# williamfgc/ROCm-MPI

Hardware: AMD Instinct MI355X
Metric: T_eff (GB/s) + weak-scaling eff., 2D diffusion 1000 steps at 1/2/4/8 MI355X (higher is better)
Workload: dtype fp64

## Files before the change

csrc/bindings/module.cpp:

```cpp
#include <pybind11/pybind11.h>
#include <pybind11/stl.h>

#include <cstdint>
#include <string>
#include <tuple>
#include <vector>

#include "rma/config.h"
#include "rma/comm.h"
#include "rma/common.h"
#include "rma/executor.h"
#include "rma/executor3d.h"
#include "rma/gather.h"
#include "rma/halo.h"
#include "rma/ipc.h"
#include "rma/kernels.h"
#include "rma/loopback.h"
#include "rma/p2p.h"
#include "rma/plan.h"
#include "rma/topology.h"
#include "rma/trace.h"

namespace py = pybind11;
using namespace rma;
// ... 134 lines not shown
        else {
          py::gil_scoped_release nogil;
          stencil2_rects_cpu(P<double>(T2), P<const double>(T), P<const double>(iCp), nx, ny,
                             r.data(), (int)r.size(), to_coef(coef));
        }
      },
      py::arg("T2"), py::arg("T"), py::arg("iCp"), py::arg("nx"), py::arg("ny"), py::arg("rects"),
      py::arg("coef"), py::arg("chunk_rows") = 8, py::arg("nontemporal") = 3,
      py::arg("stream") = 0, py::arg("gpu") = true, py::arg("unroll") = 2,
      py::arg("xcd_remap") = -1);
  m.def(
      "stencilk_rects",
      [](int K, uintptr_t T2, uintptr_t T, uintptr_t iCp, int64_t nx, int64_t ny,
         const std::vector<Rect4>& rects, const Coef4& coef, int chunk_rows, int nontemporal,
         uintptr_t stream, bool gpu, int xcd_remap, int vec, int kernel, int stages, int cols,
         bool uniform, double uniform_value) {
        auto r = to_rects(rects);
        StencilTuning tn;
        tn.cols = cols;
        tn.uniform = uniform;
        tn.uniform_value = uniform_value;
        tn.chunk_rows = chunk_rows;
        tn.nontemporal = nontemporal;
        tn.xcd_remap = xcd_remap;
        tn.vec = vec;
        tn.kernel = kernel;
        tn.stages = stages;
        if (gpu)
          stencilk_rects_gpu(K, P<double>(T2), P<const double>(T), P<const double>(iCp), nx, ny,
                             r.data(), (int)r.size(), to_coef(coef), tn, S(stream));
        else {
          const bool f5 = (kernel >= 5 && kernel <= 9) || kernel == 12 || kernel == 22;
          py::gil_scoped_release nogil;
          if (f5)
            stencilk5_rects_cpu(K, P<double>(T2), P<const double>(T), P<const double>(iCp), nx,
                                ny, r.data(), (int)r.size(), to_coef(coef));
          else
            stencilk_rects_cpu(K, P<double>(T2), P<const double>(T), P<const double>(iCp), nx,
                               ny, r.data(), (int)r.size(), to_coef(coef));
        }
      },
      py::arg("K"), py::arg("T2"), py::arg("T"), py::arg("iCp"), py::arg("nx"), py::arg("ny"),
      py::arg("rects"), py::arg("coef"), py::arg("chunk_rows") = 16, py::arg("nontemporal") = 3,
      py::arg("stream") = 0, py::arg("gpu") = true, py::arg("xcd_remap") = -1,
      py::arg("vec") = 2, py::arg("kernel") = 0, py::arg("stages") = 0, py::arg("cols") = 0,
      py::arg("uniform") = false, py::arg("uniform_value") = 0.0);
  m.def(
      "stencil3d_boxes",
      [](uintptr_t T2, uintptr_t T, uintptr_t iCp, int64_t nx, int64_t ny, int64_t nz,
         const std::vector<Box6>& boxes, const Coef5& coef, int rows, int unroll, int vec,
         int nontemporal, int chunk_z, int xcd_remap, uintptr_t stream, bool gpu, bool uniform,
         double uniform_value, bool fast_math, int xface) {
        auto b = to_boxes(boxes);
        if (gpu) {
          Stencil3DTuning tn;
          tn.fast_math = fast_math ? 1 : 0;
          tn.xface = xface;
          tn.uniform = uniform;
          tn.uniform_value = uniform_value;
          tn.rows = rows;
          tn.unroll = unroll;
// ... 397 lines not shown
      .def("set_self_via_transport", &HaloExchanger::set_self_via_transport)
      .def_property_readonly("neighbors", &HaloExchanger::neighbors)
      .def_property_readonly("bytes_sent_last", &HaloExchanger::bytes_sent_last)
      .def_property_readonly("plan_hits", &HaloExchanger::plan_hits)
      .def_property_readonly("plan_misses", &HaloExchanger::plan_misses);

  m.def("pipe_chunk_rows", &pipe_chunk_rows, py::arg("K"), py::arg("ny"),
        py::arg("canonical") = false);
  m.def("default_chunk_k", [](int K, int64_t ny) { return default_tune_k(K, ny).chunk_rows; },
        py::arg("K"), py::arg("ny"));
  m.def("plan_passes", &plan_passes, py::arg("nsteps"), py::arg("costs"));
  m.def("uniform_pass_costs", &uniform_pass_costs, py::arg("kmax"), py::arg("cells") = 0.0);
  m.def("pipe_uniform_cells", &pipe_uniform_cells, py::arg("K"), py::arg("cells"));
  m.def("default_pass_costs", &default_pass_costs, py::arg("kmax"), py::arg("fast5"),
        py::arg("cells") = 0.0);
  m.def("pipe_default_stages", &pipe_default_stages, py::arg("K"));
  m.def("pipe_default_cols", &pipe_default_cols, py::arg("K"), py::arg("stages"),
        py::arg("arith") = 0);
  m.def("pipe_has_cols", &pipe_has_cols, py::arg("K"), py::arg("stages"), py::arg("arith"),
        py::arg("cols"));
  m.def("pipe_vec", &pipe_vec, py::arg("K"), py::arg("stages"), py::arg("arith"), py::arg("nx"),
        py::arg("requested"), py::arg("aligned16") = true);
  m.def("pipe_vec_uniform", &pipe_vec_uniform, py::arg("K"), py::arg("stages"), py::arg("arith"),
        py::arg("nx"), py::arg("requested"), py::arg("aligned16") = true,
        py::arg("uniform") = false);
  m.def("pipe_max_k", []() { return kPipeMaxK; });
  m.def(
      "pass_geometry",
      [](int64_t nx, int64_t ny, int K, std::array<std::array<int, 2>, 3> nbr, bool hide,
         int64_t bwx, int64_t bwy, int64_t olx, int64_t oly) {
// ... 61 lines not shown
           py::arg("mode"), py::arg("coef"), py::arg("chunk_rows") = 4,
           py::arg("nontemporal") = 3, py::arg("kernel") = 0, py::arg("bwx") = 1,
           py::arg("bwy") = 1, py::arg("use_graph") = 0, py::arg("graph_steps") = 0,
           py::arg("halo").none(true) = nullptr, py::arg("qx") = 0, py::arg("qy") = 0,
           py::arg("dTdt") = 0, py::arg("unroll") = 4, py::arg("vec") = 2,
           py::arg("temporal") = 1, py::arg("olx") = 2, py::arg("oly") = 2,
           py::arg("chunk2") = 0, py::arg("unroll2") = 2, py::arg("fast_math") = 0,
           py::keep_alive<1, 16>())
      .def(
          "run", [](DiffusionExecutor& e, int64_t n, uintptr_t s) { e.run(n, S(s)); },
          py::arg("nsteps"), py::arg("stream"), py::call_guard<py::gil_scoped_release>())
      .def_property_readonly("parity", &DiffusionExecutor::parity)
      .def_property_readonly("steps_done", &DiffusionExecutor::steps_done)
      .def_property_readonly("passes_done", &DiffusionExecutor::passes_done)
      .def_property_readonly("fused_passes", &DiffusionExecutor::fused_passes)
      .def_property_readonly("uniform_factor", &DiffusionExecutor::uniform_factor)
      .def("rescan_factor", &DiffusionExecutor::rescan_factor,
           py::call_guard<py::gil_scoped_release>())
      .def("check_error", &DiffusionExecutor::check_error)
      .def("plan", &DiffusionExecutor::plan, py::arg("nsteps"))
      .def_property_readonly("pass_costs", &DiffusionExecutor::pass_costs)
      .def("prime", &DiffusionExecutor::prime, py::call_guard<py::gil_scoped_release>())
      .def("set_timing", &DiffusionExecutor::set_timing, py::arg("on"),
           py::call_guard<py::gil_scoped_release>())
      .def("timings",
           [](DiffusionExecutor& e) {
             std::vector<py::dict> out;
             std::vector<PassTiming> ts;
             {
               py::gil_scoped_release nogil;
// ... 151 lines not shown
```

csrc/include/rma/executor.h:

```cpp
#pragma once

#include <array>
#include <cstdint>
#include <memory>
#include <vector>

#include "rma/halo.h"
#include "rma/kernels.h"
#include "rma/plan.h"

namespace rma {

enum class Mode : int { kPerf = 0, kHide = 1, kKp = 2 };

struct ExecParams {
  Mode mode = Mode::kPerf;
  StencilCoef coef{};
  StencilTuning tune{};
  int64_t bwx = 1, bwy = 1;
  int use_graph = 0;
  int graph_steps = 0;
  int temporal = 1;
  int64_t olx = 2, oly = 2;
  StencilTuning tune2{16, 3, 0, 2, 2, -1};
// ... 19 lines not shown
  DiffusionExecutor(const DiffusionExecutor&) = delete;
  DiffusionExecutor& operator=(const DiffusionExecutor&) = delete;

  void run(int64_t nsteps, stream_t caller_stream);
  std::vector<int> plan(int64_t nsteps) const;
  const std::vector<double>& pass_costs() const { return cost_; }
  void prime();
  void set_timing(bool on);
  std::vector<PassTiming> timings();
  void set_solo(bool on);
  bool solo() const { return solo_; }
  int parity() const { return parity_; }
  int64_t steps_done() const { return steps_; }
  int64_t passes_done() const { return passes_; }
  int64_t fused_passes() const { return fused_passes_; }
  void check_error() const { check_fused_error(); }
  bool uniform_factor() const { return uniform_; }
  bool rescan_factor();
  struct DirectPeer {
    int rank = -1;
    double* T = nullptr;
    double* T2 = nullptr;
    uint64_t* flag = nullptr;
  };
  static constexpr int kDirI[8] = {-1, 0, 1, -1, 1, -1, 0, 1};
  static constexpr int kDirJ[8] = {-1, -1, -1, 0, 0, 1, 1, 1};
  void set_direct(const std::array<DirectPeer, 8>& peers, uint64_t* in_flags,
                  bool host_wait = false);
  bool direct() const { return direct_on_; }
  int64_t direct_passes() const { return direct_pass_; }
  std::vector<Rect> frame_rects() const { return frame_; }
  Rect interior_rect() const { return interior_; }
  Rect full_rect() const { return full_; }
  const PassGeom& geometry(int K);

 private:
  void enqueue_step(double* Tin, double* Tout);
  void enqueue_pass(int K, double* Tin, double* Tout);
  StencilTuning pass_tuning(int K, int part = 0) const;
  int frame_chunk_rows(int K, int interior_rows) const;
  void multi_step(int K, double* Tin, double* Tout, const double* iCp, int64_t nx, int64_t ny,
                  const Rect* rects, int n, const StencilTuning& tn, void* stream) const;
  void exchange(double* A, stream_t s);
  bool cross_pass_ = false;
  void build_graph(int64_t steps, int reps);
  void run_eager(int64_t nsteps);
  bool fast5() const;
  void scan_factor();
  bool uniform_ = false;
  double c0_ = 0.0;
  int cells_ = 0;

  double* T_;
  double* T2_;
  const double* iCp_;
  int64_t nx_, ny_;
  ExecParams p_;
// ... 64 lines not shown
```

csrc/include/rma/kernels.h:

```cpp
#pragma once

#include <cstddef>
#include <cstdint>

#include "rma/common.h"

namespace rma {

using stream_t = void*;

constexpr int kMaxRects = 8;

struct DirectStores {
  int on = 0;
  int32_t xm0 = 0, xm1 = 0, xp0 = 0, xp1 = 0;
  int32_t ym0 = 0, ym1 = 0, yp0 = 0, yp1 = 0;
  int64_t sx = 0, syr = 0;
  double* dst[8] = {};
};

struct StencilTuning {
  int chunk_rows = 4;
  int nontemporal = 3;
  int kernel = 0;
  int unroll = 4;
  int vec = 2;
  int xcd_remap = -1;
  int stages = 0;
  int cols = 0;
  uint64_t* signal = nullptr;
  int signal_rects = 0;
  int signal_chunk_rows = 0;
  const DirectStores* direct = nullptr;
  bool uniform = false;
  double uniform_value = 0.0;
};

void stencil_rects_gpu(double* T2, const double* T, const double* iCp, int64_t nx, int64_t ny,
                       const Rect* rects, int nrects, const StencilCoef& c,
                       const StencilTuning& tune, stream_t stream);
void stencil_rects_cpu(double* T2, const double* T, const double* iCp, int64_t nx, int64_t ny,
                       const Rect* rects, int nrects, const StencilCoef& c);

void stencil2_rects_gpu(double* T2, const double* T, const double* iCp, int64_t nx, int64_t ny,
                        const Rect* rects, int nrects, const StencilCoef& c,
                        const StencilTuning& tune, stream_t stream);
void stencil2_rects_cpu(double* T2, const double* T, const double* iCp, int64_t nx, int64_t ny,
// ... 6 lines not shown
                        int64_t ny, const Rect* rects, int nrects, const StencilCoef& c);
bool fast5_ok(const StencilCoef& c);
constexpr int kPipeMaxK = 24;
int pipe_default_stages(int K);
bool pipe_has(int K, int stages, int arith = 0);
bool pipe_has_cols(int K, int stages, int arith, int cols);
int pipe_default_cols(int K, int stages, int arith);
int pipe_vec(int K, int stages, int arith, int64_t nx, int requested, bool aligned16);
int pipe_vec_uniform(int K, int stages, int arith, int64_t nx, int requested, bool aligned16,
                     bool uniform);
void stencil_pipe_occupancy(int K, int stages, int arith, int V, int occ[2]);
void stencil_pipe_rects_gpu(int K, int stages, int arith, double* T2, const double* T,
                            const double* iCp, int64_t nx, int64_t ny, const Rect* rects,
                            int nrects, const StencilCoef& c, const StencilTuning& tune,
                            stream_t stream);
void stencil5_rects_cpu(double* T2, const double* T, const double* iCp, int64_t nx, int64_t ny,
                        const Rect* rects, int nrects, const StencilCoef& c);
void stencilk5_rects_cpu(int K, double* T2, const double* T, const double* iCp, int64_t nx,
                         int64_t ny, const Rect* rects, int nrects, const StencilCoef& c);

void count_differing_gpu(const double* A, int64_t n, uint64_t* out2, stream_t stream);
int64_t count_differing_cpu(const double* A, int64_t n);

constexpr int kMaxBoxes = 8;

struct Stencil3DTuning {
  int rows = 4;
  int unroll = 2;
  int vec = 2;
  int nontemporal = 3;
// ... 151 lines not shown
```

csrc/include/rma/plan.h:

```cpp
#pragma once

#include <array>
#include <cstdint>
#include <vector>

#include "rma/common.h"

namespace rma {

using Neighbors = std::array<std::array<int, 2>, 3>;

void split_rect(const Rect& out, int64_t bwx, int64_t bwy, std::vector<Rect>& frame,
                Rect& interior);
void split_rect_sides(const Rect& out, int64_t xlo, int64_t xhi, int64_t ylo, int64_t yhi,
                      std::vector<Rect>& frame, Rect& interior);

Rect owned_rect(int64_t nx, int64_t ny, int K, const Neighbors& nbr);

std::array<std::array<bool, 2>, 2> frame_sides(const Neighbors& nbr);

struct PassGeom {
  Rect out{};
  std::vector<Rect> frame;
  Rect interior{};
// ... 11 lines not shown
                       int64_t task_h = 0, int vec = 1, int bands = -1, int out_k = 0);

struct FrameLayout {
  int chunk_div = 1;
  int bands = -1;
};
FrameLayout frame_layout(int64_t ny, const Neighbors& nbr);

std::vector<double> default_pass_costs(int kmax, bool fast5, double cells = 0);
std::vector<double> uniform_pass_costs(int kmax, double cells);
int pipe_uniform_cells(int K, double cells);
void apply_cost_overrides(std::vector<double>& cost, const char* spec);

int pipe_chunk_rows(int K, int64_t ny, bool canonical);

std::vector<int> plan_passes(int64_t n, const std::vector<double>& cost);

}
```

csrc/kernels/stencil_device.h:

```cpp
#pragma once

#include <hip/hip_runtime.h>

#include <algorithm>
#include <type_traits>

#include "rma/kernels.h"

namespace rma {
namespace march {

constexpr int kWave = 64;
constexpr int kWavesPerBlock = 4;
constexpr int kBlock = kWave * kWavesPerBlock;
constexpr int64_t kColMaxWidth = 8;
typedef double dbl2 __attribute__((ext_vector_type(2)));
typedef double dbl2u __attribute__((ext_vector_type(2), aligned(8)));

template <int V>
using dbl2v = typename std::conditional<V % 2 == 0, dbl2, dbl2u>::type;

struct RectList {
  Rect r[kMaxRects];
  int64_t xa[kMaxRects];
  int64_t strips[kMaxRects];
  int64_t chunks[kMaxRects];
  int64_t block_end[kMaxRects];
  int64_t gpad[kMaxRects];
  int64_t crows[kMaxRects];
  int n;
  uint64_t* sig;
  int64_t sig_blocks;
};

template <int V, bool NTL = false>
__device__ __forceinline__ void load_row(double (&out)[V], const double* __restrict__ p) {
  if constexpr (V == 1) {
    out[0] = NTL ? __builtin_nontemporal_load(p) : *p;
  } else {
#pragma unroll
    for (int h = 0; h < V / 2; ++h) {
      const dbl2v<V>* q = reinterpret_cast<const dbl2v<V>*>(p + 2 * h);
      const dbl2v<V> t = NTL ? __builtin_nontemporal_load(q) : *q;
      out[2 * h] = t.x;
      out[2 * h + 1] = t.y;
// ... 32 lines not shown
      return;
    }
  }
#pragma unroll
  for (int i = 0; i < V; ++i) {
    if (m[i]) {
      if constexpr (NT) {
        __builtin_nontemporal_store(v[i], p + i);
      } else {
        p[i] = v[i];
      }
    }
  }
}

__device__ __forceinline__ int64_t xcd_remap(int64_t b, int64_t nwg) {
  constexpr int64_t kXcd = 8;
  if (nwg < kXcd) return b;
  const int64_t q = nwg / kXcd, r = nwg % kXcd;
  const int64_t xcd = b % kXcd, slot = b / kXcd;
  return (xcd < r ? xcd * (q + 1) : r * (q + 1) + (xcd - r) * q) + slot;
}

__device__ __forceinline__ int64_t xcd_remap_after(int64_t b, int64_t nwg, int64_t first) {
  return b < first ? b : first + xcd_remap(b - first, nwg - first);
}

__device__ __forceinline__ void signal_block_done(uint64_t* sig, int64_t nblocks) {
  __syncthreads();
  if (threadIdx.x == 0) {
    const uint64_t old =
        __hip_atomic_fetch_add(sig, (uint64_t)1, __ATOMIC_ACQ_REL, __HIP_MEMORY_SCOPE_AGENT);
    if ((int64_t)old + 1 == nblocks) {
      __hip_atomic_store(sig, (uint64_t)0, __ATOMIC_RELAXED, __HIP_MEMORY_SCOPE_AGENT);
      __hip_atomic_store(sig + 1, (uint64_t)1, __ATOMIC_RELEASE, __HIP_MEMORY_SCOPE_SYSTEM);
    }
  }
}

__device__ __forceinline__ void signal_wave_done(uint64_t* sig, int64_t nwaves) {
// ... 139 lines not shown
```

csrc/kernels/stencil_pipe.h:

```cpp
#pragma once

#include <hip/hip_runtime.h>

#include <type_traits>

#include "pipe_arith.h"
#include "rma/common.h"
#include "rma/hip_check.h"
#include "rma/kernels.h"
#include "stencil_device.h"

namespace rma {
namespace pipe {
using namespace march;

template <int K, int S>
struct Plan {
  static constexpr int H = (K + S - 1) / S;
  static constexpr int HL = K - (S - 1) * H;
  static constexpr int R = K + S - 1;
  static_assert(S >= 1 && HL >= 1 && HL <= H, "bad stage split");
};

template <int V>
// ... 126 lines not shown
  static_assert(V != 6 || Uni, "6 cells per lane: the uniform-factor variant only");
  constexpr bool kU6 = pipe_u6<K, S, Ar, Uni>();
  constexpr int NST = staging_rows<K, S, Ar, Uni>();
  using G = Geo<K, S, V, C>;
  constexpr int H = P::H, HL = P::HL, R = ring_rows<K, S, V>();
  constexpr int M = kRegG ? 0 : mirror_rows<K, S, V, Canon, C>();
  constexpr bool kDelay = kDelayedRing<V>;
  static_assert(V != 5 || (C == 1 && Ar == kArFast5), "5 cells per lane: fast5, one column wave");
  constexpr int W = G::W, WB = G::WB, D = G::D;
  constexpr int kStep = G::kStep;
  constexpr int NH = S > 1 ? S - 1 : 1;
  const int wv = __builtin_amdgcn_readfirstlane(threadIdx.x >> 6);
  const int col = C > 1 ? wv / S : 0;
  const int stage = wv % S;
  const int lane = threadIdx.x & (kWave - 1);
  const int64_t sig_first = L.sig ? L.sig_blocks : 0;
  const int64_t b = remap ? xcd_remap_after(blockIdx.x, gridDim.x, sig_first) : (int64_t)blockIdx.x;
  int ri = 0;
  while (ri < L.n - 1 && b >= L.block_end[ri]) ++ri;
  const int64_t lb = b - (ri ? L.block_end[ri - 1] : 0);
  const int64_t strip = lb % L.strips[ri], chunk = lb / L.strips[ri];
  const Rect r = L.r[ri];
  const int64_t xs = L.xa[ri] + strip * kStep;
  const int64_t crows = L.crows[ri];
  const int64_t ya = r.y0 + chunk * crows;
  const int64_t yb = min(r.y1, ya + crows);

  const int lo = col > 0 ? G::Hp : 0, hi = col < C - 1 ? D + G::Hp : W;
  const int64_t xw = xs + (int64_t)col * D;
  const int64_t x = xw + (int64_t)lane * V;
  bool m[V], cin[V];
#pragma unroll
  for (int v = 0; v < V; ++v) {
    const int p = lane * V + v, pb = col * D + p;
    m[v] = pb >= K && pb < K + kStep && p >= lo && p < hi && x + v >= r.x0 && x + v < r.x1;
    cin[v] = (x + v >= 1) && (x + v <= nx - 2);
// ... 392 lines not shown
      else if constexpr (S > 2)
        run(std::false_type{}, std::false_type{}, XINc);
    }
  };
  if constexpr (Uni) {
    if (xin)
      role(std::true_type{});
    else
      role(std::false_type{});
  } else {
    role(std::true_type{});
  }
  if constexpr (kGlds) {
    if (stage == 0) asm volatile("s_waitcnt vmcnt(0)" ::: "memory");
  }
  if (b < sig_first) signal_block_done(L.sig, L.sig_blocks);
}

template <int K, int S, int V, int Ar, int C, bool Dir = false, bool Uni = false>
__global__ __launch_bounds__(kWave * S * C) __attribute__((amdgpu_waves_per_eu(
    kernel_waves<K, S, V, Ar, C, Uni>()))) void pipe_kernel(double* __restrict__ T2,
                                                           const double* __restrict__ T,
                                                           const double* __restrict__ iCp,
                                                           int64_t nx, int64_t ny, RectList L,
                                                           StencilCoef k, int chunk_rows,
                                                           int remap, DirectStores D, double c0) {
  pipe_body<K, S, V, Ar, C, Dir, Uni>(T2, T, iCp, nx, ny, L, k, chunk_rows, remap, D, c0);
}

template <int V, int Ar, int C>
constexpr bool has_direct() {
// ... 10 lines not shown
  const double* T;
  const double* iCp;
  int64_t nx, ny;
  const Rect* rects;
  int nrects;
  StencilCoef k;
  int chunk_rows, remap;
  hipStream_t stream;
  uint64_t* sig = nullptr;
  int sig_rects = 0;
  int sig_chunk_rows = 0;
  const DirectStores* direct = nullptr;
  int* occupancy = nullptr;
  int uniform = 0;
  double c0 = 0.0;
};

template <int K, int S, int V, int Ar, int C = 1, bool WithUni = false>
void launch(const PipeLaunch& a) {
  if (a.occupancy) {
    const int bs = kWave * S * C;
    a.occupancy[0] = a.occupancy[1] = 0;
    if constexpr (V == 6) {
      RMA_HIP_CHECK(hipOccupancyMaxActiveBlocksPerMultiprocessor(
          &a.occupancy[0], pipe_kernel<K, S, V, Ar, C, false, true>, bs, 0));
    } else {
      RMA_HIP_CHECK(hipOccupancyMaxActiveBlocksPerMultiprocessor(
          &a.occupancy[0], pipe_kernel<K, S, V, Ar, C, false>, bs, 0));
      if constexpr (has_direct<V, Ar, C>())
        RMA_HIP_CHECK(hipOccupancyMaxActiveBlocksPerMultiprocessor(
            &a.occupancy[1], pipe_kernel<K, S, V, Ar, C, true>, bs, 0));
    }
    return;
  }
  int rows_buf[kMaxRects] = {};
  const int* rows = nullptr;
  if (a.sig_rects > 0 && a.sig_chunk_rows > 0) {
    for (int i = 0; i < a.sig_rects && i < kMaxRects; ++i) rows_buf[i] = a.sig_chunk_rows;
    rows = rows_buf;
  }
  RectList L;
  const int64_t blocks =
      plan_strip_tasks(L, a.rects, a.nrects, V, a.chunk_rows, K, Geo<K, S, V, C>::WB, rows);
  static_assert(Geo<K, S, V, C>::kStep == (Geo<K, S, V, C>::WB - 2 * K) / V * V, "strip step");
  if (L.n == 0) return;
  RMA_CHECK_ARG(blocks < (int64_t(1) << 31), "grid too large: " << blocks << " blocks");
  if (a.sig) {
    int ns = 0;
    for (int i = 0; i < a.sig_rects; ++i) ns += a.rects[i].empty() ? 0 : 1;
    RMA_CHECK_ARG(ns > 0, "signalling launch without a non-empty signal rect");
    L.sig = a.sig;
    L.sig_blocks = L.block_end[ns - 1];
  }
  const dim3 grid((unsigned)blocks), block(kWave * S * C);
  if constexpr (V == 6) {
    static_assert(WithUni && has_uniform<V, Ar, C>(), "6 cells per lane: uniform factor");
    RMA_CHECK_ARG(a.uniform && !(a.direct && a.direct->on),
                  "6 cells per lane without a uniform 1/Cp or with direct-store halos");
    pipe_kernel<K, S, V, Ar, C, false, true><<<grid, block, 0, a.stream>>>(
        a.T2, a.T, a.iCp, a.nx, a.ny, L, a.k, a.chunk_rows, a.remap, DirectStores{}, a.c0);
  } else {
// ... 56 lines not shown
```

csrc/kernels/stencil_pipe.hip:

```cpp
#include <hip/hip_runtime.h>

#include <cmath>

#include "rma/hip_check.h"
#include "rma/kernels.h"
#include "lab_hooks.h"
#include "stencil_pipe.h"

namespace rma {


void stencil_pipe_occupancy(int K, int stages, int arith, int V, int occ[2]) {
  const int S = stages > 0 ? stages : pipe_default_stages(K);
  RMA_CHECK_ARG(pipe_has(K, S, arith), "no pipelined kernel for K=" << K << " S=" << S
                                                                   << " arithmetic " << arith);
  pipe::PipeLaunch a{nullptr, nullptr, nullptr, 0, 0, nullptr, 0, StencilCoef{}, 1, 0, nullptr};
  a.occupancy = occ;
  occ[0] = occ[1] = 0;
  if (V != 5)
    (void)(pipe::dispatch_r20(K, S, V, arith, a) || pipe::dispatch_r24(K, S, V, arith, a) ||
           pipe::dispatch_r(K, S, V, arith, a) ||
           pipe::dispatch_a(K, S, V, arith, a) ||
           pipe::dispatch_b(K, S, V, arith, a) || pipe::dispatch_c(K, S, V, arith, a));
}

void stencil_pipe_rects_gpu(int K, int stages, int arith, double* T2, const double* T,
                            const double* iCp, int64_t nx, int64_t ny, const Rect* rects,
                            int nrects, const StencilCoef& c, const StencilTuning& tune,
                            stream_t stream) {
  const int S = stages > 0 ? stages : pipe_default_stages(K);
  RMA_CHECK_ARG(K >= 1 && K <= kPipeMaxK,
                "pipelined K-step kernel: 1 <= K <= " << kPipeMaxK << ", got " << K);
  RMA_CHECK_ARG(pipe_has(K, S, arith), "no pipelined kernel instantiated for K=" << K << " S=" << S
                                                                             << " arithmetic " << arith);
  const bool canonical = arith == pipe::kArCanon;
  RMA_CHECK_ARG(canonical || fast5_ok(c),
                "the fast5 arithmetic folds dy^-2/dx^-2 into one factor: needs lam != 0 and "
                "finite coefficients");
// ... 38 lines not shown
    }
    a.direct = &D;
  }
  if (tune.uniform && !a.direct) {
    a.uniform = 1;
    a.c0 = tune.uniform_value;
  }
  if (tune.signal || tune.signal_rects > 0) {
    RMA_CHECK_ARG(tune.signal_rects >= 1 && tune.signal_rects < nrects,
                  "signal rects " << tune.signal_rects << " of " << nrects);
    a.sig = tune.signal;
    a.sig_rects = tune.signal_rects;
    RMA_CHECK_ARG(tune.signal_chunk_rows >= 0, "signal_chunk_rows=" << tune.signal_chunk_rows);
    a.sig_chunk_rows = tune.signal_chunk_rows;
  }
  bool ok = C == 1 && V != 5 &&
            (pipe::dispatch_r20(K, S, V, arith, a) || pipe::dispatch_r24(K, S, V, arith, a) ||
           pipe::dispatch_r(K, S, V, arith, a) ||
             pipe::dispatch_a(K, S, V, arith, a) ||
             pipe::dispatch_b(K, S, V, arith, a) || pipe::dispatch_c(K, S, V, arith, a));
  if (!ok) {
    if (!lab_hooks().pipe)
      lab_missing("this pipelined kernel variant (stages / arithmetic / cols / 5 cells per lane)");
    ok = lab_hooks().pipe(K, S, V, C, arith, a);
  }
  RMA_CHECK_ARG(ok, "pipelined kernel K=" << K << " S=" << S << " V=" << V << " C=" << C
                                           << " arithmetic=" << arith << " not instantiated");
  RMA_HIP_LAUNCH_CHECK();
}

}
```

csrc/runtime/config.cpp:

```cpp
#include "rma/config.h"

#include <cerrno>
#include <cmath>
#include <cstdlib>
#include <cstring>
#include <sstream>
#include <vector>

#include "rma/common.h"

namespace rma {

const char* const kDiagKeys[] = {
    "skip_exchange",
    "exec_streams",
    "exec_verbose",
    "no_prime",
    "no_lag",
    "no_halo_cross",
    "no_halo_merged",
    "no_halo_batch",
    "frame_sides",
    "frame_chunk_div",
    "frame_aligned",
    "frame_bands",
    "no_frame_fill",
    "pipe_fast",
    "pass_costs",
    "uniform_factor",
    "pipe_cells",
    "rccl_data_blocking",
    "rccl_graph",
    "no_ipc_graph",
    "hostname",
    "rccl_fallback",
    "bench_rc_dir",
    "bench_n1_cache",
    "bench_check_raise",
    "bench_check_corrupt",
    "bench_window_corrupt",
    "bench_field_corrupt",
    "bench_rccl_log_dir",
    nullptr};

namespace {
// ... 74 lines not shown
```

csrc/runtime/executor.cpp:

```cpp
#include "rma/executor.h"

#include <hip/hip_runtime.h>

#include <algorithm>
#include <array>
#include <chrono>
#include <cmath>
#include <cstdio>
#include <cstdlib>
#include <cstring>
#include <limits>
#include <mutex>
#include <string>
#include <thread>
#include <utility>

#include "rma/config.h"
#include "rma/hip_check.h"
#include "rma/trace.h"

namespace rma {

namespace {
hipStream_t S(void* p) { return reinterpret_cast<hipStream_t>(p); }
// ... 133 lines not shown
    RMA_HIP_CHECK(hipStreamCreateWithPriority(&lo, hipStreamNonBlocking, least));
    RMA_HIP_CHECK(hipStreamCreateWithPriority(&hi, hipStreamNonBlocking, greatest));
  }
  if (diag_flag("exec_verbose"))
    fprintf(stderr, "[executor] priority range least=%d greatest=%d mode=%s hi=%p lo=%p\n", least,
            greatest, mode.c_str(), (void*)hi, (void*)lo);
  s_hi_ = hi;
  s_lo_ = lo;
  for (void** e : {&e_hi_, &e_lo_, &e_in_, &e_fr_})
    RMA_HIP_CHECK(hipEventCreateWithFlags(reinterpret_cast<hipEvent_t*>(e), hipEventDisableTiming));
  lag_ = !diag_flag("no_lag");
  const std::string fu = env_choice("RMA_EXEC_FUSED", "auto|0|1", "auto");
  fused_ = fu == "auto" ? 2 : fu == "1" ? 1 : 0;
  fused_timeout_s_ = env_double("RMA_EXEC_FUSED_TIMEOUT", 60.0, 1e-9, 1e6);
  {
    int dev = 0, cus = 0;
    RMA_HIP_CHECK(hipGetDevice(&dev));
    RMA_HIP_CHECK(hipDeviceGetAttribute(&cus, hipDeviceAttributeMultiprocessorCount, dev));
    cus_ = cus > 0 ? cus : 256;
  }
    if (fused_ && p_.mode == Mode::kHide) {
      RMA_HIP_CHECK(hipMalloc(reinterpret_cast<void**>(&sig_), 2 * sizeof(uint64_t)));
      RMA_HIP_CHECK(hipMemsetAsync(sig_, 0, 2 * sizeof(uint64_t), S(s_lo_)));
      RMA_HIP_CHECK(hipStreamSynchronize(S(s_lo_)));
      RMA_HIP_CHECK(hipHostMalloc(reinterpret_cast<void**>(&ferr_host_), sizeof(uint32_t),
                                  hipHostMallocMapped));
      *ferr_host_ = 0;
      RMA_HIP_CHECK(
          hipHostGetDevicePointer(reinterpret_cast<void**>(&ferr_dev_), ferr_host_, 0));
    }
// ... 235 lines not shown
                                   const StencilTuning& tn, void* stream) const {
  if (K == 2 && tn.kernel < 5) {
    stencil2_rects_gpu(Tout, Tin, iCp, nx, ny, rects, n, p_.coef, tn, stream);
    return;
  }
  if (!uniform_) {
    stencilk_rects_gpu(K, Tout, Tin, iCp, nx, ny, rects, n, p_.coef, tn, stream);
    return;
  }
  StencilTuning tu = tn;
  tu.uniform = true;
  tu.uniform_value = c0_;
  stencilk_rects_gpu(K, Tout, Tin, iCp, nx, ny, rects, n, p_.coef, tu, stream);
}

bool DiffusionExecutor::fused_pass_ok(const PassGeom& g, const StencilTuning& tn) const {
  if (!sig_ || !g.aligned || tn.kernel < 9 || g.interior.empty()) return false;
  int nf = 0;
  for (const Rect& r : g.frame) nf += r.empty() ? 0 : 1;
  if (nf == 0 || (int)g.frame.size() + 1 > kMaxRects) return false;
  return fused_ == 1 || g.tasks() > 2 * (int64_t)cus_;
}

template <typename Launch>
void DiffusionExecutor::enqueue_fused(const std::vector<Rect>& frame, const Rect& interior,
                                      StencilTuning tn, double* Tout, void* const* ev,
                                      Launch&& launch) {
  ++fused_passes_;
  auto rec = [&](int i, void* stream) {
    if (ev[4]) RMA_HIP_CHECK(hipEventRecord(E(ev[i]), S(stream)));
// ... 237 lines not shown
    if (dr) flags_write_gpu(dout_, direct_pass_ + 1, stream);
  };
  void* ev[5] = {nullptr, nullptr, nullptr, nullptr, nullptr};
  if (timing_) {
    for (auto& e : ev) e = tevent();
    if (ev[4]) tk_.push_back(K);
  }
  auto rec = [&](int i, void* stream) {
    if (ev[4]) RMA_HIP_CHECK(hipEventRecord(E(ev[i]), S(stream)));
  };
  if (p_.mode == Mode::kPerf) {
    TraceRange tr("rma.pass.perf");
    rec(0, s_lo_);
    rec(3, s_lo_);
    dwait(s_lo_);
    multi_step(K, Tin, Tout, iCp_, nx_, ny_, &g.out, 1, with_direct(tn), s_lo_);
    rec(4, s_lo_);
    rec(1, s_lo_);
    if (da)
      dpost(s_lo_);
    else
      exchange(Tout, s_lo_);
    rec(2, s_lo_);
    if (ev[4]) tseq_.push_back(1);
    return;
  }
  if (da && (!dr || g.frame.empty() || g.tasks() <= 2 * (int64_t)cus_)) {
    TraceRange tr("rma.pass.direct");
    RMA_HIP_CHECK(hipStreamWaitEvent(S(s_lo_), E(e_hi_), 0));
    rec(0, s_lo_);
    rec(3, s_lo_);
// ... 11 lines not shown
      multi_step(K, Tin, Tout, iCp_, nx_, ny_, &g.out, 1, with_direct(tn), s_lo_);
    }
    rec(4, s_lo_);
    rec(1, s_lo_);
    dpost(s_lo_);
    rec(2, s_lo_);
    RMA_HIP_CHECK(hipEventRecord(E(e_lo_), S(s_lo_)));
    if (ev[4]) tseq_.push_back(1);
    return;
  }
  if (g.frame.empty()) {
    TraceRange tr("rma.pass.hide");
    RMA_HIP_CHECK(hipStreamWaitEvent(S(s_lo_), E(e_hi_), 0));
    rec(0, s_lo_);
    rec(3, s_lo_);
    multi_step(K, Tin, Tout, iCp_, nx_, ny_, &g.interior, 1, tn, s_lo_);
    rec(4, s_lo_);
    rec(1, s_lo_);
    exchange(Tout, s_lo_);
    rec(2, s_lo_);
    RMA_HIP_CHECK(hipEventRecord(E(e_lo_), S(s_lo_)));
    if (ev[4]) tseq_.push_back(1);
    return;
  }
  if (fused_pass_ok(g, tn)) {
    TraceRange tr("rma.pass.fused");
    enqueue_fused(g.frame, g.interior, with_direct(tn), Tout, ev,
                  [&](const Rect* rs, int n, const StencilTuning& t) {
                    multi_step(K, Tin, Tout, iCp_, nx_, ny_, rs, n, t, s_lo_);
                  });
    return;
// ... 278 lines not shown
```

csrc/runtime/plan.cpp:

```cpp
#include "rma/config.h"
#include "rma/plan.h"

#include <algorithm>
#include <cmath>
#include <cstdlib>
#include <limits>
#include <string>

namespace rma {

void split_rect_sides(const Rect& out, int64_t xlo, int64_t xhi, int64_t ylo, int64_t yhi,
                      std::vector<Rect>& frame, Rect& interior) {
  RMA_CHECK_ARG(xlo >= 0 && xhi >= 0 && ylo >= 0 && yhi >= 0,
                "frame widths " << xlo << "," << xhi << "," << ylo << "," << yhi);
  frame.clear();
  const int64_t xi0 = out.x0 + xlo, xi1 = out.x1 - xhi;
  const int64_t yi0 = out.y0 + ylo, yi1 = out.y1 - yhi;
  if (xi0 >= xi1 || yi0 >= yi1) {
    interior = {0, 0, 0, 0};
    if (!out.empty()) frame.push_back(out);
    return;
  }
  interior = {xi0, xi1, yi0, yi1};
  if (ylo > 0) frame.push_back({out.x0, out.x1, out.y0, yi0});
// ... 156 lines not shown
  if (ny < 12288) {
    if (canonical) return K <= 12 ? 128 : 256;
    return K <= 9 ? 256 : K <= 16 ? 128 : 256;
  }
  if (ny < 24576) {
    if (canonical) return K <= 9 ? 256 : K <= 12 ? 512 : 384;
    return K <= 4 ? 768 : K <= 9 ? 1536 : 512;
  }
  if (ny < 32768) {
    if (K <= 9) return 0;
    return canonical ? 512 : 768;
  }
  return 0;
}

std::vector<double> default_pass_costs(int kmax, bool fast5, double cells) {
  RMA_CHECK_ARG(kmax >= 1 && kmax <= 24, "kmax=" << kmax << " (tables cover 1..24)");
  int t = kTables - 1;
  if (cells > 0) {
    double best = 1e300;
    for (int i = 0; i < kTables; ++i) {
      const double d = std::fabs(std::log(cells / kTileCells[i]));
      if (d < best) {
        best = d;
        t = i;
      }
    }
  }
  std::vector<double> c(kmax + 1, kInf);
  for (int K = 1; K <= kmax; ++K) c[K] = fast5 ? kFast5[t][K] : kCanon[t][K];
// ... 62 lines not shown
```

rocm_mpi_amd/config.py:

```python
from __future__ import annotations

import os

DIAG_KEYS = {
    "skip_exchange": "every halo exchange skipped (WRONG multi-rank results)",
    "exec_streams": "pool | lofirst | hifirst | plain: executor stream creation",
    "exec_verbose": "print the executor's stream priorities",
    "no_prime": "no kernel priming at executor construction",
    "no_lag": "every pass waits for the previous exchange",
    "no_halo_cross": "one-step passes: one RCCL group per dimension",
    "no_halo_merged": "x+y neighbours: one group per dimension (C++ and Python)",
    "no_halo_batch": "one pack / unpack launch per plane",
    "frame_sides": "all: frame rects on every side once any neighbour exists",
    "frame_chunk_div": "N: aligned frame tasks of 1/N the interior's rows",
    "frame_aligned": "0 | 1: force the frame layout",
    "frame_bands": "task | ol: force the aligned y-band height",
    "no_frame_fill": "frame bands not filled into the interior",
    "pipe_fast": "pipe | pipe5: the LDS-ring fast kernel at every depth",
    "pass_costs": "K:cost/K:cost/...: planner cost overrides",
    "uniform_factor": "off: the 1/Cp field path also where 1/Cp is one value",
    "pipe_cells": "4 | 6: uniform passes at four cells everywhere / six on every tile",
    "rccl_data_blocking": "blocking RCCL data path of a non-blocking communicator",
    "rccl_graph": "allow hipGraph capture over RCCL",
    "no_ipc_graph": "refuse hipGraph capture over the IPC transport",
    "hostname": "node name for the local-rank exchange (tests)",
    "rccl_fallback": "an RCCL init failure falls back to the staged transport",
    "bench_rc_dir": "bench.py: every rank writes its exit status into this directory",
    "bench_n1_cache": "bench.py: path of the N = 1 record",
    "bench_check_raise": "bench.py: before | after: injected halo-check failure",
    "bench_check_corrupt": "bench.py: corrupt one halo-check cell",
    "bench_window_corrupt": "bench.py: corrupt one headline-window cell",
    "bench_field_corrupt": "bench.py: nan | hot | cold: one bad timed-field cell",
    "bench_rccl_log_dir": "bench.py: RCCL log directory of the link probe",
}


# ... 33 lines not shown
```

Baseline: 94740.

## Split pipelined stencil regions into graded row bands to balance the tail

Single-rank pipelined K>=20 passes on tall grids now split the region into up to three row bands with descending rows per task (6144/768/192). Each band gets its own XCD remap range. The aim is to shrink the tail imbalance where the last large tasks leave compute units idle, using occupancy-derived slot counts. It adds host-side planning per launch and only applies when no neighbours exist, so multi-rank runs are unchanged.

```diff
diff --git a/csrc/bindings/module.cpp b/csrc/bindings/module.cpp
--- a/csrc/bindings/module.cpp
+++ b/csrc/bindings/module.cpp
@@ -172,9 +172,13 @@
       [](int K, uintptr_t T2, uintptr_t T, uintptr_t iCp, int64_t nx, int64_t ny,
          const std::vector<Rect4>& rects, const Coef4& coef, int chunk_rows, int nontemporal,
          uintptr_t stream, bool gpu, int xcd_remap, int vec, int kernel, int stages, int cols,
-         bool uniform, double uniform_value) {
+         bool uniform, double uniform_value, const std::vector<int>& rect_rows, int bands) {
         auto r = to_rects(rects);
         StencilTuning tn;
+        if (!rect_rows.empty() && rect_rows.size() != r.size())
+          throw std::invalid_argument("rect_rows: one entry per rect");
+        tn.rect_rows = rect_rows.empty() ? nullptr : rect_rows.data();
+        tn.bands = bands;
         tn.cols = cols;
         tn.uniform = uniform;
         tn.uniform_value = uniform_value;
@@ -202,7 +206,8 @@
       py::arg("rects"), py::arg("coef"), py::arg("chunk_rows") = 16, py::arg("nontemporal") = 3,
       py::arg("stream") = 0, py::arg("gpu") = true, py::arg("xcd_remap") = -1,
       py::arg("vec") = 2, py::arg("kernel") = 0, py::arg("stages") = 0, py::arg("cols") = 0,
-      py::arg("uniform") = false, py::arg("uniform_value") = 0.0);
+      py::arg("uniform") = false, py::arg("uniform_value") = 0.0,
+      py::arg("rect_rows") = std::vector<int>{}, py::arg("bands") = 0);
   m.def(
       "stencil3d_boxes",
       [](uintptr_t T2, uintptr_t T, uintptr_t iCp, int64_t nx, int64_t ny, int64_t nz,
@@ -630,6 +635,64 @@
   m.def("pipe_uniform_cells", &pipe_uniform_cells, py::arg("K"), py::arg("cells"));
   m.def("default_pass_costs", &default_pass_costs, py::arg("kmax"), py::arg("fast5"),
         py::arg("cells") = 0.0);
+  m.def(
+      "plan_row_bands",
+      [](int64_t y0, int64_t y1, int64_t strips, int64_t slots, const std::array<int, 3>& rows,
+         int uniform_rows, double fill) {
+        std::vector<std::tuple<int64_t, int64_t, int>> out;
+        for (const RowBand& b : plan_row_bands(y0, y1, strips, slots, rows, uniform_rows, fill))
+          out.emplace_back(b.y0, b.y1, b.rows);
+        return out;
+      },
+      py::arg("y0"), py::arg("y1"), py::arg("strips"), py::arg("slots"), py::arg("rows"),
+      py::arg("uniform_rows"), py::arg("fill") = kBandFill);
+  m.def("pipe_band_rows", &pipe_band_rows, py::arg("K"), py::arg("ny"));
+  m.def("pipe_strip_count", &pipe_strip_count, py::arg("x0"), py::arg("x1"), py::arg("K"),
+        py::arg("V"));
+  m.def(
+      "parse_task_rows",
+      [](const std::string& spec) {
+        std::array<int, 3> rows{{0, 0, 0}};
+        double fill = kBandFill;
+        bool uniform = false;
+        const bool forced = parse_task_rows(spec, rows, fill, uniform);
+        return std::make_tuple(forced, uniform, rows, fill);
+      },
+      py::arg("spec"));
+  m.def(
+      "pipe_task_map",
+      [](const std::vector<Rect4>& rects, int V, int chunk_rows, int halo, int64_t sw_block,
+         const std::vector<int>& rect_rows, int bands, int sig_rects, int remap) {
+        auto r = to_rects(rects);
+        if (!rect_rows.empty() && rect_rows.size() != r.size())
+          throw std::invalid_argument("rect_rows: one entry per rect");
+        const int* rr = rect_rows.empty() ? nullptr : rect_rows.data();
+        const int64_t n = pipe_task_map(r.data(), (int)r.size(), V, chunk_rows, halo, sw_block, rr,
+                                        bands, sig_rects, remap, nullptr);
+        std::vector<int64_t> flat((size_t)(3 * n));
+        pipe_task_map(r.data(), (int)r.size(), V, chunk_rows, halo, sw_block, rr, bands,
+                      sig_rects, remap, flat.data());
+        std::vector<std::tuple<int64_t, int64_t, int64_t>> out;
+        for (int64_t b = 0; b < n; ++b)
+          out.emplace_back(flat[3 * b], flat[3 * b + 1], flat[3 * b + 2]);
+        return out;
+      },
+      py::arg("rects"), py::arg("V"), py::arg("chunk_rows"), py::arg("halo"),
+      py::arg("sw_block") = 0, py::arg("rect_rows") = std::vector<int>{}, py::arg("bands") = 0,
+      py::arg("sig_rects") = 0, py::arg("remap") = 1);
+  m.def("pipe_last_launch", []() {
+    int64_t v[2] = {0, 0};
+    pipe_last_launch(v);
+    return std::make_tuple(v[0], v[1]);
+  });
+  m.def(
+      "stencil_pipe_occupancy",
+      [](int K, int stages, int arith, int V) {
+        int occ[2] = {0, 0};
+        stencil_pipe_occupancy(K, stages, arith, V, occ);
+        return std::make_tuple(occ[0], occ[1]);
+      },
+      py::arg("K"), py::arg("stages"), py::arg("arith"), py::arg("V"));
   m.def("pipe_default_stages", &pipe_default_stages, py::arg("K"));
   m.def("pipe_default_cols", &pipe_default_cols, py::arg("K"), py::arg("stages"),
         py::arg("arith") = 0);
@@ -721,6 +784,16 @@
       .def_property_readonly("steps_done", &DiffusionExecutor::steps_done)
       .def_property_readonly("passes_done", &DiffusionExecutor::passes_done)
       .def_property_readonly("fused_passes", &DiffusionExecutor::fused_passes)
+      .def_property_readonly("graded_passes", &DiffusionExecutor::graded_passes)
+      .def(
+          "row_bands",
+          [](DiffusionExecutor& e, int K, const Rect4& r) {
+            std::vector<std::tuple<int64_t, int64_t, int>> out;
+            for (const RowBand& b : e.row_bands(K, to_rects({r})[0]))
+              out.emplace_back(b.y0, b.y1, b.rows);
+            return out;
+          },
+          py::arg("K"), py::arg("rect"))
       .def_property_readonly("uniform_factor", &DiffusionExecutor::uniform_factor)
       .def("rescan_factor", &DiffusionExecutor::rescan_factor,
            py::call_guard<py::gil_scoped_release>())
diff --git a/csrc/include/rma/executor.h b/csrc/include/rma/executor.h
--- a/csrc/include/rma/executor.h
+++ b/csrc/include/rma/executor.h
@@ -57,6 +57,8 @@
   int64_t steps_done() const { return steps_; }
   int64_t passes_done() const { return passes_; }
   int64_t fused_passes() const { return fused_passes_; }
+  int64_t graded_passes() const { return graded_passes_; }
+  std::vector<RowBand> row_bands(int K, const Rect& r);
   void check_error() const { check_fused_error(); }
   bool uniform_factor() const { return uniform_; }
   bool rescan_factor();
@@ -84,6 +86,17 @@
   int frame_chunk_rows(int K, int interior_rows) const;
   void multi_step(int K, double* Tin, double* Tout, const double* iCp, int64_t nx, int64_t ny,
                   const Rect* rects, int n, const StencilTuning& tn, void* stream) const;
+  void launch_region(int K, double* Tin, double* Tout, const Rect& r, const StencilTuning& tn,
+                     void* stream);
+  std::vector<RowBand> region_bands(int K, const Rect& r, const StencilTuning& tn);
+  int rows_mode_ = 0;
+  std::array<int, 3> rows_forced_{{0, 0, 0}};
+  double rows_fill_ = kBandFill;
+  struct BandSlots {
+    int stages = 0, arith = 0, vec = 0, slots = 0;
+  };
+  std::vector<BandSlots> band_slots_;
+  int64_t graded_passes_ = 0;
   void exchange(double* A, stream_t s);
   bool cross_pass_ = false;
   void build_graph(int64_t steps, int reps);
diff --git a/csrc/include/rma/kernels.h b/csrc/include/rma/kernels.h
--- a/csrc/include/rma/kernels.h
+++ b/csrc/include/rma/kernels.h
@@ -31,6 +31,8 @@
   uint64_t* signal = nullptr;
   int signal_rects = 0;
   int signal_chunk_rows = 0;
+  const int* rect_rows = nullptr;
+  int bands = 0;
   const DirectStores* direct = nullptr;
   bool uniform = false;
   double uniform_value = 0.0;
@@ -67,6 +69,10 @@
                             const double* iCp, int64_t nx, int64_t ny, const Rect* rects,
                             int nrects, const StencilCoef& c, const StencilTuning& tune,
                             stream_t stream);
+int64_t pipe_task_map(const Rect* rects, int nrects, int V, int chunk_rows, int halo,
+                      int64_t sw_block, const int* rect_rows, int bands, int sig_rects, int remap,
+                      int64_t* out);
+void pipe_last_launch(int64_t out[2]);
 void stencil5_rects_cpu(double* T2, const double* T, const double* iCp, int64_t nx, int64_t ny,
                         const Rect* rects, int nrects, const StencilCoef& c);
 void stencilk5_rects_cpu(int K, double* T2, const double* T, const double* iCp, int64_t nx,
diff --git a/csrc/include/rma/plan.h b/csrc/include/rma/plan.h
--- a/csrc/include/rma/plan.h
+++ b/csrc/include/rma/plan.h
@@ -2,6 +2,7 @@
 
 #include <array>
 #include <cstdint>
+#include <string>
 #include <vector>
 
 #include "rma/common.h"
@@ -49,6 +50,19 @@
 
 int pipe_chunk_rows(int K, int64_t ny, bool canonical);
 
+struct RowBand {
+  int64_t y0 = 0, y1 = 0;
+  int rows = 0;
+};
+constexpr double kBandFill = 2.0;
+std::vector<RowBand> plan_row_bands(int64_t y0, int64_t y1, int64_t strips, int64_t slots,
+                                    const std::array<int, 3>& rows, int uniform_rows,
+                                    double fill = kBandFill);
+std::array<int, 3> pipe_band_rows(int K, int64_t ny);
+int64_t pipe_strip_count(int64_t x0, int64_t x1, int K, int V);
+bool parse_task_rows(const std::string& spec, std::array<int, 3>& rows, double& fill,
+                     bool& uniform);
+
 std::vector<int> plan_passes(int64_t n, const std::vector<double>& cost);
 
 }
diff --git a/csrc/kernels/stencil_device.h b/csrc/kernels/stencil_device.h
--- a/csrc/kernels/stencil_device.h
+++ b/csrc/kernels/stencil_device.h
@@ -29,6 +29,7 @@
   int64_t gpad[kMaxRects];
   int64_t crows[kMaxRects];
   int n;
+  int nbands;
   uint64_t* sig;
   int64_t sig_blocks;
 };
@@ -91,7 +92,7 @@
   }
 }
 
-__device__ __forceinline__ int64_t xcd_remap(int64_t b, int64_t nwg) {
+__host__ __device__ __forceinline__ int64_t xcd_remap(int64_t b, int64_t nwg) {
   constexpr int64_t kXcd = 8;
   if (nwg < kXcd) return b;
   const int64_t q = nwg / kXcd, r = nwg % kXcd;
@@ -99,8 +100,42 @@
   return (xcd < r ? xcd * (q + 1) : r * (q + 1) + (xcd - r) * q) + slot;
 }
 
-__device__ __forceinline__ int64_t xcd_remap_after(int64_t b, int64_t nwg, int64_t first) {
+__host__ __device__ __forceinline__ int64_t xcd_remap_after(int64_t b, int64_t nwg,
+                                                            int64_t first) {
   return b < first ? b : first + xcd_remap(b - first, nwg - first);
+}
+
+struct StripTask {
+  int ri;
+  int64_t strip, chunk;
+};
+__host__ __device__ __forceinline__ StripTask locate_strip_task(const RectList& L, int64_t blk,
+                                                                int64_t nwg, int remap) {
+  const int64_t first = L.sig ? L.sig_blocks : 0;
+  int64_t b = blk;
+  if (remap && b >= first) {
+    int64_t s = first, e = nwg;
+    if (L.nbands > 1) {
+      const int fb = L.n - L.nbands;
+      const int64_t bs = fb ? L.block_end[fb - 1] : 0;
+      if (b < bs) {
+        e = bs;
+      } else {
+        int i = fb;
+        while (i < L.n - 1 && b >= L.block_end[i]) ++i;
+        s = i ? L.block_end[i - 1] : 0;
+        e = L.block_end[i];
+      }
+    }
+    b = s + xcd_remap(b - s, e - s);
+  }
+  StripTask t;
+  t.ri = 0;
+  while (t.ri < L.n - 1 && b >= L.block_end[t.ri]) ++t.ri;
+  const int64_t lb = b - (t.ri ? L.block_end[t.ri - 1] : 0);
+  t.strip = lb % L.strips[t.ri];
+  t.chunk = lb / L.strips[t.ri];
+  return t;
 }
 
 __device__ __forceinline__ void signal_block_done(uint64_t* sig, int64_t nblocks) {
diff --git a/csrc/kernels/stencil_pipe.h b/csrc/kernels/stencil_pipe.h
--- a/csrc/kernels/stencil_pipe.h
+++ b/csrc/kernels/stencil_pipe.h
@@ -164,12 +164,9 @@
   const int col = C > 1 ? wv / S : 0;
   const int stage = wv % S;
   const int lane = threadIdx.x & (kWave - 1);
-  const int64_t sig_first = L.sig ? L.sig_blocks : 0;
-  const int64_t b = remap ? xcd_remap_after(blockIdx.x, gridDim.x, sig_first) : (int64_t)blockIdx.x;
-  int ri = 0;
-  while (ri < L.n - 1 && b >= L.block_end[ri]) ++ri;
-  const int64_t lb = b - (ri ? L.block_end[ri - 1] : 0);
-  const int64_t strip = lb % L.strips[ri], chunk = lb / L.strips[ri];
+  const StripTask task = locate_strip_task(L, blockIdx.x, gridDim.x, remap);
+  const int ri = task.ri;
+  const int64_t strip = task.strip, chunk = task.chunk;
   const Rect r = L.r[ri];
   const int64_t xs = L.xa[ri] + strip * kStep;
   const int64_t crows = L.crows[ri];
@@ -592,7 +589,7 @@
   if constexpr (kGlds) {
     if (stage == 0) asm volatile("s_waitcnt vmcnt(0)" ::: "memory");
   }
-  if (b < sig_first) signal_block_done(L.sig, L.sig_blocks);
+  if (L.sig && (int64_t)blockIdx.x < L.sig_blocks) signal_block_done(L.sig, L.sig_blocks);
 }
 
 template <int K, int S, int V, int Ar, int C, bool Dir = false, bool Uni = false>
@@ -633,6 +630,9 @@
   int* occupancy = nullptr;
   int uniform = 0;
   double c0 = 0.0;
+  const int* rect_rows = nullptr;
+  int bands = 0;
+  int64_t* planned = nullptr;
 };
 
 template <int K, int S, int V, int Ar, int C = 1, bool WithUni = false>
@@ -658,12 +658,22 @@
     for (int i = 0; i < a.sig_rects && i < kMaxRects; ++i) rows_buf[i] = a.sig_chunk_rows;
     rows = rows_buf;
   }
+  if (a.rect_rows) {
+    for (int i = 0; i < a.nrects && i < kMaxRects; ++i)
+      if (a.rect_rows[i] > 0) rows_buf[i] = a.rect_rows[i];
+    rows = rows_buf;
+  }
   RectList L;
   const int64_t blocks =
       plan_strip_tasks(L, a.rects, a.nrects, V, a.chunk_rows, K, Geo<K, S, V, C>::WB, rows);
   static_assert(Geo<K, S, V, C>::kStep == (Geo<K, S, V, C>::WB - 2 * K) / V * V, "strip step");
   if (L.n == 0) return;
   RMA_CHECK_ARG(blocks < (int64_t(1) << 31), "grid too large: " << blocks << " blocks");
+  L.nbands = a.bands;
+  if (a.planned) {
+    a.planned[0] = blocks;
+    a.planned[1] = L.nbands;
+  }
   if (a.sig) {
     int ns = 0;
     for (int i = 0; i < a.sig_rects; ++i) ns += a.rects[i].empty() ? 0 : 1;
diff --git a/csrc/kernels/stencil_pipe.hip b/csrc/kernels/stencil_pipe.hip
--- a/csrc/kernels/stencil_pipe.hip
+++ b/csrc/kernels/stencil_pipe.hip
@@ -1,5 +1,6 @@
 #include <hip/hip_runtime.h>
 
+#include <atomic>
 #include <cmath>
 
 #include "rma/hip_check.h"
@@ -22,6 +23,50 @@
            pipe::dispatch_r(K, S, V, arith, a) ||
            pipe::dispatch_a(K, S, V, arith, a) ||
            pipe::dispatch_b(K, S, V, arith, a) || pipe::dispatch_c(K, S, V, arith, a));
+}
+
+namespace {
+std::atomic<int64_t> g_last_blocks{0}, g_last_bands{0};
+}
+
+void pipe_last_launch(int64_t out[2]) {
+  out[0] = g_last_blocks.load();
+  out[1] = g_last_bands.load();
+}
+
+int64_t pipe_task_map(const Rect* rects, int nrects, int V, int chunk_rows, int halo,
+                      int64_t sw_block, const int* rect_rows, int bands, int sig_rects, int remap,
+                      int64_t* out) {
+  RMA_CHECK_ARG(nrects >= 0 && nrects <= kMaxRects, "nrects=" << nrects);
+  RMA_CHECK_ARG(V >= 1 && chunk_rows >= 1 && halo >= 0, "V=" << V << " chunk_rows=" << chunk_rows
+                                                             << " halo=" << halo);
+  RMA_CHECK_ARG((sw_block > 0 ? sw_block : 64 * V) - 2 * halo >= V, "strip narrower than its halo");
+  RMA_CHECK_ARG(sig_rects >= 0 && bands >= 0 && bands <= nrects - sig_rects,
+                "bands=" << bands << " sig_rects=" << sig_rects << " of " << nrects << " rects");
+  int ns = 0;
+  for (int i = 0; i < nrects; ++i) {
+    RMA_CHECK_ARG(!rect_rows || rect_rows[i] >= 0, "rect_rows[" << i << "]");
+    RMA_CHECK_ARG(i < nrects - bands || !rects[i].empty(), "band rect " << i << " is empty");
+    if (i < sig_rects && !rects[i].empty()) ++ns;
+  }
+  march::RectList L;
+  const int64_t blocks =
+      march::plan_strip_tasks(L, rects, nrects, V, chunk_rows, halo, sw_block, rect_rows);
+  if (L.n == 0) return 0;
+  L.nbands = bands;
+  static uint64_t dummy[2];
+  if (ns > 0) {
+    L.sig = dummy;
+    L.sig_blocks = L.block_end[ns - 1];
+  }
+  if (out)
+    for (int64_t b = 0; b < blocks; ++b) {
+      const march::StripTask t = march::locate_strip_task(L, b, blocks, remap);
+      out[3 * b] = t.ri;
+      out[3 * b + 1] = t.strip;
+      out[3 * b + 2] = t.chunk;
+    }
+  return blocks;
 }
 
 void stencil_pipe_rects_gpu(int K, int stages, int arith, double* T2, const double* T,
@@ -90,6 +135,20 @@
     RMA_CHECK_ARG(tune.signal_chunk_rows >= 0, "signal_chunk_rows=" << tune.signal_chunk_rows);
     a.sig_chunk_rows = tune.signal_chunk_rows;
   }
+  if (tune.rect_rows)
+    for (int i = 0; i < nrects; ++i)
+      RMA_CHECK_ARG(tune.rect_rows[i] >= 0, "rect_rows[" << i << "]=" << tune.rect_rows[i]);
+  a.rect_rows = tune.rect_rows;
+  if (tune.bands > 0) {
+    RMA_CHECK_ARG(tune.bands <= nrects - a.sig_rects,
+                  "bands=" << tune.bands << " of " << nrects << " rects, " << a.sig_rects
+                           << " of them signal rects");
+    for (int i = nrects - tune.bands; i < nrects; ++i)
+      RMA_CHECK_ARG(!rects[i].empty(), "band rect " << i << " is empty");
+    a.bands = tune.bands;
+  }
+  int64_t planned[2] = {0, 0};
+  a.planned = planned;
   bool ok = C == 1 && V != 5 &&
             (pipe::dispatch_r20(K, S, V, arith, a) || pipe::dispatch_r24(K, S, V, arith, a) ||
            pipe::dispatch_r(K, S, V, arith, a) ||
@@ -103,6 +162,8 @@
   RMA_CHECK_ARG(ok, "pipelined kernel K=" << K << " S=" << S << " V=" << V << " C=" << C
                                            << " arithmetic=" << arith << " not instantiated");
   RMA_HIP_LAUNCH_CHECK();
+  g_last_blocks.store(planned[0]);
+  g_last_bands.store(planned[1]);
 }
 
 }
diff --git a/csrc/runtime/config.cpp b/csrc/runtime/config.cpp
--- a/csrc/runtime/config.cpp
+++ b/csrc/runtime/config.cpp
@@ -29,6 +29,7 @@
     "pass_costs",
     "uniform_factor",
     "pipe_cells",
+    "task_rows",
     "rccl_data_blocking",
     "rccl_graph",
     "no_ipc_graph",
diff --git a/csrc/runtime/executor.cpp b/csrc/runtime/executor.cpp
--- a/csrc/runtime/executor.cpp
+++ b/csrc/runtime/executor.cpp
@@ -171,6 +171,12 @@
   fused_ = fu == "auto" ? 2 : fu == "1" ? 1 : 0;
   fused_timeout_s_ = env_double("RMA_EXEC_FUSED_TIMEOUT", 60.0, 1e-9, 1e6);
   {
+    bool uni = false;
+    const bool forced = parse_task_rows(diag_value("task_rows"), rows_forced_, rows_fill_, uni);
+    rows_mode_ = forced ? 2 : uni ? 1 : 0;
+    band_slots_.assign(kPipeMaxK + 1, BandSlots{});
+  }
+  {
     int dev = 0, cus = 0;
     RMA_HIP_CHECK(hipGetDevice(&dev));
     RMA_HIP_CHECK(hipDeviceGetAttribute(&cus, hipDeviceAttributeMultiprocessorCount, dev));
@@ -436,6 +442,54 @@
   stencilk_rects_gpu(K, Tout, Tin, iCp, nx, ny, rects, n, p_.coef, tu, stream);
 }
 
+std::vector<RowBand> DiffusionExecutor::region_bands(int K, const Rect& r,
+                                                     const StencilTuning& tn) {
+  const std::vector<RowBand> single{{r.y0, r.y1, tn.chunk_rows}};
+  bool alone = true;
+  for (int d = 0; d < 2; ++d) alone = alone && real_nbr_[d][0] < 0 && real_nbr_[d][1] < 0;
+  const std::array<int, 3> rows = rows_mode_ == 2 ? rows_forced_ : pipe_band_rows(K, ny_);
+  if (tn.kernel < 9 || !alone || r.empty() || tn.direct || tn.signal || tn.signal_rects > 0 ||
+      rows_mode_ == 1 || (rows_mode_ == 0 && p_.chunk_rows2 > 0) || rows[0] <= 0)
+    return single;
+  const int arith = tn.kernel - 9;
+  const int S = tn.stages > 0 ? tn.stages : pipe_default_stages(K);
+  const int V = pipe_vec_uniform(K, tn.stages, arith, nx_, tn.vec, true, uniform_);
+  if (V < 1 || 64 * V - 2 * K < V) return single;
+  BandSlots& bs = band_slots_[K];
+  if (bs.slots == 0 || bs.stages != S || bs.arith != arith || bs.vec != V) {
+    int occ[2] = {0, 0};
+    stencil_pipe_occupancy(K, S, arith, V, occ);
+    bs = {S, arith, V, cus_ * std::max(1, occ[0])};
+  }
+  return plan_row_bands(r.y0, r.y1, pipe_strip_count(r.x0, r.x1, K, V), bs.slots, rows,
+                        tn.chunk_rows, rows_fill_);
+}
+
+std::vector<RowBand> DiffusionExecutor::row_bands(int K, const Rect& r) {
+  return region_bands(K, r, pass_tuning(K, 0));
+}
+
+void DiffusionExecutor::launch_region(int K, double* Tin, double* Tout, const Rect& r,
+                                      const StencilTuning& tn, void* stream) {
+  const std::vector<RowBand> bands = region_bands(K, r, tn);
+  if (bands.size() < 2 || bands.size() > (size_t)kMaxRects) {
+    multi_step(K, Tin, Tout, iCp_, nx_, ny_, &r, 1, tn, stream);
+    return;
+  }
+  Rect rs[kMaxRects];
+  int rows[kMaxRects] = {};
+  int n = 0;
+  for (const RowBand& b : bands) {
+    rs[n] = {r.x0, r.x1, b.y0, b.y1};
+    rows[n++] = b.rows;
+  }
+  StencilTuning t = tn;
+  t.rect_rows = rows;
+  t.bands = n;
+  multi_step(K, Tin, Tout, iCp_, nx_, ny_, rs, n, t, stream);
+  ++graded_passes_;
+}
+
 bool DiffusionExecutor::fused_pass_ok(const PassGeom& g, const StencilTuning& tn) const {
   if (!sig_ || !g.aligned || tn.kernel < 9 || g.interior.empty()) return false;
   int nf = 0;
@@ -703,7 +757,7 @@
     rec(0, s_lo_);
     rec(3, s_lo_);
     dwait(s_lo_);
-    multi_step(K, Tin, Tout, iCp_, nx_, ny_, &g.out, 1, with_direct(tn), s_lo_);
+    launch_region(K, Tin, Tout, g.out, with_direct(tn), s_lo_);
     rec(4, s_lo_);
     rec(1, s_lo_);
     if (da)
@@ -745,7 +799,7 @@
     RMA_HIP_CHECK(hipStreamWaitEvent(S(s_lo_), E(e_hi_), 0));
     rec(0, s_lo_);
     rec(3, s_lo_);
-    multi_step(K, Tin, Tout, iCp_, nx_, ny_, &g.interior, 1, tn, s_lo_);
+    launch_region(K, Tin, Tout, g.interior, tn, s_lo_);
     rec(4, s_lo_);
     rec(1, s_lo_);
     exchange(Tout, s_lo_);
diff --git a/csrc/runtime/plan.cpp b/csrc/runtime/plan.cpp
--- a/csrc/runtime/plan.cpp
+++ b/csrc/runtime/plan.cpp
@@ -194,6 +194,78 @@
   return 0;
 }
 
+std::vector<RowBand> plan_row_bands(int64_t y0, int64_t y1, int64_t strips, int64_t slots,
+                                    const std::array<int, 3>& rows, int uniform_rows,
+                                    double fill) {
+  RMA_CHECK_ARG(y1 > y0 && strips >= 1 && slots >= 1 && uniform_rows >= 1,
+                "row bands of [" << y0 << ", " << y1 << "), " << strips << " strips, " << slots
+                                 << " slots, " << uniform_rows << " rows per task");
+  RMA_CHECK_ARG(fill > 0.0 && fill <= 64.0, "band fill " << fill);
+  const std::vector<RowBand> single{{y0, y1, uniform_rows}};
+  if (rows[0] <= 0 || (rows[1] <= 0 && rows[2] <= 0)) return single;
+  int prev = rows[0];
+  for (int i = 1; i < 3; ++i) {
+    RMA_CHECK_ARG(rows[i] >= 0 && (rows[i] == 0 || rows[i] < prev),
+                  "band rows " << rows[0] << "/" << rows[1] << "/" << rows[2]
+                               << " must descend");
+    if (rows[i] > 0) prev = rows[i];
+  }
+  const int64_t R = y1 - y0;
+  const int64_t chunks = std::max<int64_t>(1, (int64_t)std::ceil(fill * (double)slots / (double)strips));
+  auto tail = [&](int r) { return r > 0 ? std::min(chunks * r, R / 4) : (int64_t)0; };
+  const int64_t t1 = tail(rows[1]), t2 = tail(rows[2]);
+  const int64_t n0 = (R - t1 - t2) / rows[0] * rows[0];
+  if (n0 <= 0) return single;
+  const int64_t rest = R - n0;
+  const int64_t n1 = rows[1] <= 0 ? 0 : rows[2] <= 0 ? rest : (rest - t2) / rows[1] * rows[1];
+  const int64_t n2 = rest - n1;
+  std::vector<RowBand> b{{y0, y0 + n0, rows[0]}};
+  if (n1 > 0) b.push_back({y0 + n0, y0 + n0 + n1, rows[1]});
+  if (n2 > 0) b.push_back({y0 + n0 + n1, y1, rows[2]});
+  return b;
+}
+
+std::array<int, 3> pipe_band_rows(int K, int64_t ny) {
+  if (K >= 20 && ny >= 98304) return {6144, 768, 192};
+  return {0, 0, 0};
+}
+
+int64_t pipe_strip_count(int64_t x0, int64_t x1, int K, int V) {
+  RMA_CHECK_ARG(V >= 1 && K >= 1 && 64 * V - 2 * K >= V && x1 > x0,
+                "strips of [" << x0 << ", " << x1 << ") at K=" << K << " V=" << V);
+  const int64_t step = (64 * V - 2 * K) / V * V;
+  const int64_t xs = x0 - K, xa = xs - (((xs % V) + V) % V);
+  return (x1 - (xa + K) + step - 1) / step;
+}
+
+bool parse_task_rows(const std::string& spec, std::array<int, 3>& rows, double& fill,
+                     bool& uniform) {
+  uniform = spec == "uniform";
+  if (spec.empty() || uniform) return false;
+  double v[4] = {0, 0, 0, kBandFill};
+  int n = 0;
+  size_t pos = 0;
+  bool ok = true;
+  while (ok && pos <= spec.size()) {
+    const size_t end = std::min(spec.find('/', pos), spec.size());
+    const std::string item = spec.substr(pos, end - pos);
+    char* e = nullptr;
+    const double x = std::strtod(item.c_str(), &e);
+    ok = n < 4 && !item.empty() && e && *e == '\0' && std::isfinite(x) && x >= 0 && x < (1 << 30);
+    if (ok) v[n++] = x;
+    pos = end + 1;
+  }
+  ok = ok && n >= 3 && v[0] >= 1 && v[0] == std::floor(v[0]) && v[1] == std::floor(v[1]) &&
+       v[2] == std::floor(v[2]) && v[3] > 0 && v[3] <= 64;
+  ok = ok && (v[1] > 0 || v[2] > 0) && (v[1] == 0 || v[1] < v[0]) &&
+       (v[2] == 0 || v[2] < (v[1] > 0 ? v[1] : v[0]));
+  RMA_CHECK_ARG(ok, "RMA_DIAG task_rows=" << spec
+                        << " (uniform | r0/r1/r2[/fill], rows per task descending)");
+  rows = {(int)v[0], (int)v[1], (int)v[2]};
+  fill = v[3];
+  return true;
+}
+
 std::vector<double> default_pass_costs(int kmax, bool fast5, double cells) {
   RMA_CHECK_ARG(kmax >= 1 && kmax <= 24, "kmax=" << kmax << " (tables cover 1..24)");
   int t = kTables - 1;
diff --git a/rocm_mpi_amd/config.py b/rocm_mpi_amd/config.py
--- a/rocm_mpi_amd/config.py
+++ b/rocm_mpi_amd/config.py
@@ -20,6 +20,7 @@
     "pass_costs": "K:cost/K:cost/...: planner cost overrides",
     "uniform_factor": "off: the 1/Cp field path also where 1/Cp is one value",
     "pipe_cells": "4 | 6: uniform passes at four cells everywhere / six on every tile",
+    "task_rows": "uniform | r0/r1/r2[/fill]: graded task rows off / forced on any tile",
     "rccl_data_blocking": "blocking RCCL data path of a non-blocking communicator",
     "rccl_graph": "allow hipGraph capture over RCCL",
     "no_ipc_graph": "refuse hipGraph capture over the IPC transport",
```

Result: faster. 97560 (median of 6 runs) (+3.0%).
